# jamie8johnson/cqs

Measured on AMD Instinct MI355X. Metric: queries/sec @k=20 (brute-force cosine scan + top-k, 768-d fp32), higher is better.
Workload: dtype f32; 1 GPU; BASELINE configs[1]: 1000000 x 768 fp32 unit vectors, 1 query per step, brute-force cosine top-20; mode=single, rows_per_gpu=1000000, total_rows=1000000, dim=768, k=20, parallelism=single GPU, ranks_seen=1

## Files before the change

cqs_amd/csrc/scan_bf16.hip:

```cpp
#include "scan_bf16.h"
#include "scan_i8.h"
#include "f32_score.h"
#include "launch_util.h"
#include "rank_sort.h"
#include "scan_gemv_device.h"
#include "select_device.h"
#include "shadow_build_device.h"
#include "tail_plan.h"
#include "tail_prefix.h"

namespace cqs {

static_assert(kShadowKMax == kMaxK, "shadow k' policy and the select agree on max k");

__device__ __forceinline__ float key_score(uint64_t key) {
    const uint32_t ok = (uint32_t)(key >> 32);
    return __uint_as_float((ok & 0x80000000u) ? (ok ^ 0x80000000u) : ~ok);
}

__global__ __launch_bounds__(256) void shadow_build_kernel(const float* __restrict__ rows, uint16_t* __restrict__ shadow,
                                                           uint64_t row0, uint64_t n_rows, uint32_t dim, double gamma,
                                                           unsigned long long* __restrict__ stats) {
    const int lane = threadIdx.x & 63;
    const uint64_t waves = (uint64_t)gridDim.x * (blockDim.x >> 6);
    for (uint64_t r = (uint64_t)blockIdx.x * (blockDim.x >> 6) + (threadIdx.x >> 6); r < n_rows; r += waves) {
        shadow_build_row(rows + (row0 + r) * dim, shadow + (row0 + r) * dim, dim, gamma, stats, lane);
    }
}

hipError_t launch_shadow_build(const float* rows, uint16_t* shadow, uint64_t row0, uint64_t n_rows, uint32_t dim,
                               double gamma, unsigned long long* stats, hipStream_t st) {
    if (n_rows == 0) return hipSuccess;
    const uint64_t blocks = (n_rows + 3u) / 4u;
    hipLaunchKernelGGL(shadow_build_kernel, dim3((uint32_t)(blocks < 8192u ? blocks : 8192u)), dim3(256), 0, st, rows,
                       shadow, row0, n_rows, dim, gamma, stats);
    return hipGetLastError();
}

__global__ __launch_bounds__(64) void shadow_bound_kernel(const float* __restrict__ q, uint32_t dim, double r_max,
                                                          double norm_max, float* __restrict__ bq) {
    const uint32_t lane = threadIdx.x;
    const float v = wave_shadow_bound(q + (size_t)blockIdx.x * dim, dim, r_max, norm_max, lane);
    if (lane == 0) bq[blockIdx.x] = v;
}

hipError_t launch_shadow_bound(const float* q, uint32_t b, uint32_t dim, double r_max, double norm_max, float* bq,
                               hipStream_t st) {
    if (b == 0) return hipSuccess;
    if (b > kShadowMaxQ) return hipErrorInvalidValue;
    hipLaunchKernelGGL(shadow_bound_kernel, dim3(b), dim3(64), 0, st, q, dim, r_max, norm_max, bq);
    return hipGetLastError();
}

struct Bf16ScanParams {
    const uint16_t* rows;
    uint32_t n, n_pad, dim;
    const float* q;
    float* scores;
    const uint32_t* keep;
    uint32_t mode;
    float thr;
    uint32_t nq;
    uint32_t* work;
    TaskTiers tiers;
    uint32_t n_tasks;
    float* gmax;
    uint64_t* gaux;
    const float* bq;
    uint32_t keep_stride;
    uint8_t slot[kMaxGemvQ];
};

template <int NCH, int BQ, int RI, bool NT, bool FULL, bool PQ>
__global__ __launch_bounds__(256) void scan_bf16_kernel(const Bf16ScanParams p) {
    constexpr int NV = RI * BQ;
    constexpr int LPV = 64 / NV;
    const int lane = threadIdx.x & 63;
    const uint32_t n = p.n, dim = p.dim;

    uint32_t coff[NCH];
    f4 qa[BQ][NCH], qb[BQ][NCH];
#pragma unroll
    for (int c = 0; c < NCH; ++c) {
        const uint32_t idx = (uint32_t)c * 512u + (uint32_t)lane * 8u;
        const bool in = FULL || idx < dim;
        coff[c] = in ? idx : dim - 8u;
#pragma unroll
        for (int b = 0; b < BQ; ++b) {
            const float* qp = p.q + (size_t)((uint32_t)b < p.nq ? b : 0) * dim + coff[c];
            const f4 va = *(const f4*)qp, vb = *(const f4*)(qp + 4);
            qa[b][c] = in ? va : (f4)(0.f);
            qb[b][c] = in ? vb : (f4)(0.f);
        }
    }

    const uint32_t last = n - 1u;
    const uint32_t nwords = (n + 31u) / 32u;
    const uint32_t n_tasks = p.n_tasks;
    const uint32_t wpb = blockDim.x >> 6;
    const uint32_t total_waves = gridDim.x * wpb;
    const uint32_t wave_id = (uint32_t)__builtin_amdgcn_readfirstlane((int)(blockIdx.x * wpb + (threadIdx.x >> 6)));
    const bool use_queue = n_tasks > total_waves;
    const uint32_t zero = opaque_zero();

    const char* const rows_b = (const char*)p.rows;
    const uint32_t row_bytes = dim * 2u;
    auto load_rows = [&](uint32_t base, int j, u4 (&x)[RI][NCH]) {
#pragma unroll
        for (int r = 0; r < RI; ++r) {
            uint32_t row = base + (uint32_t)(RI * j + r);
            row = row > last ? last : row;
            const char* rp = rows_b + (uint64_t)row * row_bytes;
#pragma unroll
            for (int c = 0; c < NCH; ++c) {
                const u4* src = (const u4*)(rp + coff[c] * 2u);
                if (NT) x[r][c] = __builtin_nontemporal_load(src);
                else x[r][c] = *src;
            }
        }
        __builtin_amdgcn_sched_barrier(0);
    };
    auto reduce_rows = [&](int j, u4 (&x)[RI][NCH], float (&sc)[BQ]) {
        f2 acc2[NV];
#pragma unroll
        for (int i = 0; i < NV; ++i) acc2[i] = (f2)(0.f);
#pragma unroll
        for (int r = 0; r < RI; ++r)
#pragma unroll
            for (int c = 0; c < NCH; ++c) {
                const u4 w = x[r][c];
                const f2 x0 = {bf_lo(w.x), bf_hi(w.x)}, x1 = {bf_lo(w.y), bf_hi(w.y)};
                const f2 x2 = {bf_lo(w.z), bf_hi(w.z)}, x3 = {bf_lo(w.w), bf_hi(w.w)};
#pragma unroll
                for (int b = 0; b < BQ; ++b) {
                    f2 a = acc2[b * RI + r];
                    a = __builtin_elementwise_fma(x0, __builtin_shufflevector(qa[b][c], qa[b][c], 0, 1), a);
                    a = __builtin_elementwise_fma(x1, __builtin_shufflevector(qa[b][c], qa[b][c], 2, 3), a);
                    a = __builtin_elementwise_fma(x2, __builtin_shufflevector(qb[b][c], qb[b][c], 0, 1), a);
                    a = __builtin_elementwise_fma(x3, __builtin_shufflevector(qb[b][c], qb[b][c], 2, 3), a);
                    acc2[b * RI + r] = a;
                }
            }
        float acc[NV];
#pragma unroll
        for (int i = 0; i < NV; ++i) acc[i] = acc2[i].x + acc2[i].y;
        treduce<NV>(acc, lane);
#pragma unroll
        for (int b = 0; b < BQ; ++b) {
            const float t = __shfl(acc[0], (b * RI + (lane % RI)) * LPV, 64);
            if (lane / RI == j) sc[b] = t;
        }
    };
    uint64_t qmask[PQ ? BQ : 1];
    auto epilogue = [&](uint32_t cur, uint32_t base, uint32_t trows, uint64_t mask, float (&sc)[BQ]) {
        const uint32_t row = base + (uint32_t)lane;
        const bool live_all = (uint32_t)lane < trows && ((mask >> lane) & 1ull);
#pragma unroll
        for (int b = 0; b < BQ; ++b) {
            const bool live = PQ ? (uint32_t)lane < trows && ((qmask[PQ ? b : 0] >> lane) & 1ull) : live_all;
            float s = sc[b];
            if (!live || !(__builtin_fabsf(s) <= 3.4028234664e38f)) s = -INFINITY;
            else if (p.mode == 1u && (uint32_t)b < p.nq) {
                float t = s + p.bq[b];
                t = t < 0.f ? 0.f : (t > 1.f ? 1.f : t);
                if (!(t >= p.thr)) s = -INFINITY;
            }
            if ((uint32_t)b >= p.nq) continue;
            if ((uint32_t)lane < trows && row < p.n_pad) p.scores[(size_t)b * p.n_pad + row] = s;
            const float gm = wave_max64(s);
            if (lane == 0) p.gmax[(size_t)b * n_tasks + cur] = gm;
            if (p.gaux) {
                const uint32_t arg = (uint32_t)__builtin_ctzll(__ballot(s == gm));
                const float sec = wave_max64(((uint32_t)lane == arg) ? -INFINITY : s);
                if (lane == 0) p.gaux[(size_t)b * n_tasks + cur] = ((uint64_t)arg << 32) | (uint64_t)__float_as_uint(sec);
            }
        }
    };
    auto task_mask = [&](uint32_t base, uint32_t trows) -> uint64_t {
        const uint64_t all = trows == 64u ? ~0ull : ((1ull << trows) - 1ull);
        uint64_t mask = all;
        if (base + trows > n) mask = (base >= n) ? 0ull : (all >> (trows - (n - base)));
        if constexpr (PQ) {
            const uint32_t w = base / 32u;
            uint64_t any = 0ull;
#pragma unroll
            for (int b = 0; b < BQ; ++b) {
                uint64_t m = 0ull;
                if ((uint32_t)b < p.nq) {
                    const kc32* kp = (const kc32*)(p.keep + (size_t)p.slot[b] * p.keep_stride);
                    const uint32_t w0 = (w < nwords) ? kp[w] : 0u;
                    const uint32_t w1 = (w + 1u < nwords) ? kp[w + 1u] : 0u;
                    m = mask & ((((uint64_t)w1 << 32) | (uint64_t)w0) >> (base & 31u));
                }
                const uint32_t mlo = __builtin_amdgcn_readfirstlane((uint32_t)m);
                const uint32_t mhi = __builtin_amdgcn_readfirstlane((uint32_t)(m >> 32));
                qmask[b] = ((uint64_t)mhi << 32) | mlo;
                any |= qmask[b];
            }
            return any;
        }
        if (p.keep) {
            const uint32_t w = base / 32u;
            const uint32_t w0 = (w < nwords) ? p.keep[w] : 0u;
            const uint32_t w1 = (w + 1u < nwords) ? p.keep[w + 1u] : 0u;
            mask &= (((uint64_t)w1 << 32) | (uint64_t)w0) >> (base & 31u);
        }
        const uint32_t mlo = __builtin_amdgcn_readfirstlane((uint32_t)mask);
        const uint32_t mhi = __builtin_amdgcn_readfirstlane((uint32_t)(mask >> 32));
        return ((uint64_t)mhi << 32) | mlo;
    };

    u4 x[RI][NCH];
    uint32_t cur = wave_id;
    while (cur < n_tasks) {
        uint32_t trows;
        const uint32_t base = p.tiers.locate(cur, trows);
        const uint64_t mask = task_mask(base, trows);
        uint32_t ticket = 0;
        if (use_queue && lane == 0) ticket = atomicAdd(p.work + zero, 1u);
        float sc[BQ];
#pragma unroll
        for (int b = 0; b < BQ; ++b) sc[b] = -INFINITY;
        const int nb = (int)(trows / (uint32_t)RI);
        for (int j = 0; j < nb; ++j) {
            const uint32_t m = (uint32_t)(mask >> (RI * j)) & ((1u << RI) - 1u);
            if (m == 0u) continue;
            load_rows(base, j, x);
            reduce_rows(j, x, sc);
        }
        epilogue(cur, base, trows, mask, sc);
        cur = use_queue ? total_waves + (uint32_t)__builtin_amdgcn_readfirstlane(ticket) : n_tasks;
    }
}

#ifndef CQS_BF16_ONE_SHOT
#define CQS_BF16_ONE_SHOT 24u
#endif
#ifndef CQS_BF16_BLOCKS_PER_CU
#define CQS_BF16_BLOCKS_PER_CU 2u
#endif

template <int NCH, int BQ, int RI, bool PQ>
static hipError_t launch_bf16(const ScanArgs& a, const uint16_t* shadow, const float* bq, uint32_t q0, uint32_t nq,
                              uint32_t work_slot, hipStream_t st) {
    Bf16ScanParams p;
    fill_gemv_pass(p, a, q0, nq, PQ);
    p.rows = shadow;
    p.work = a.work + work_slot;
    p.bq = bq + q0;
    const bool one_shot = p.n_tasks <= a.n_cu * 4u * CQS_BF16_ONE_SHOT;
    const uint32_t wpb = 4u;
    const uint32_t blocks = one_shot ? (p.n_tasks + wpb - 1u) / wpb : a.n_cu * CQS_BF16_BLOCKS_PER_CU;
    const dim3 grid(blocks), block(64u * wpb);
    const bool full = (a.dim == (uint32_t)NCH * 512u);
    for_nt_full(a.nontemporal, full, [&](auto nt_c, auto full_c) {
        hipLaunchKernelGGL((scan_bf16_kernel<NCH, BQ, RI, decltype(nt_c)::value, decltype(full_c)::value, PQ>), grid, block, 0, st, p);
    });
    return hipGetLastError();
}

template <int NCH, bool PQ>
static hipError_t launch_bf16_groups(const ScanArgs& a, const uint16_t* shadow, const float* bq, hipStream_t st) {
    uint32_t done = 0, slot = 0;
    while (done < a.b) {
        const uint32_t left = a.b - done;
        hipError_t e;
        uint32_t g;
        if constexpr (NCH <= 2) {
            if (left >= 5) { g = left < 8u ? left : 8u; e = launch_bf16<NCH, 8, 2, PQ>(a, shadow, bq, done, g, slot, st); }
            else if (left >= 4) { g = 4; e = launch_bf16<NCH, 4, 4, PQ>(a, shadow, bq, done, g, slot, st); }
            else if (left >= 2) { g = 2; e = launch_bf16<NCH, 2, 8, PQ>(a, shadow, bq, done, g, slot, st); }
            else { g = 1; e = launch_bf16<NCH, 1, 16, PQ>(a, shadow, bq, done, g, slot, st); }
        } else {
            if (left >= 2) { g = 2; e = launch_bf16<NCH, 2, 4, PQ>(a, shadow, bq, done, g, slot, st); }
            else { g = 1; e = launch_bf16<NCH, 1, 8, PQ>(a, shadow, bq, done, g, slot, st); }
        }
        if (e != hipSuccess) return e;
        done += g;
        slot = (slot + 1u) % kWorkWords;
    }
    return hipSuccess;
}

hipError_t launch_scan_bf16(const ScanArgs& a, const uint16_t* shadow, const float* bq, hipStream_t st) {
    if (a.b == 0 || a.n == 0) return hipSuccess;
    if (a.b > kShadowMaxQ || a.dim % 8u != 0u || a.dim > kShadowMaxDim || a.group_tasks != 1u) return hipErrorInvalidValue;
    if (a.keep_tab && !keep_tab_ok(a)) return hipErrorInvalidValue;
    switch ((a.dim + 511u) / 512u) {
        case 1: return a.keep_tab ? launch_bf16_groups<1, true>(a, shadow, bq, st) : launch_bf16_groups<1, false>(a, shadow, bq, st);
        case 2: return a.keep_tab ? launch_bf16_groups<2, true>(a, shadow, bq, st) : launch_bf16_groups<2, false>(a, shadow, bq, st);
        case 3: return a.keep_tab ? launch_bf16_groups<3, true>(a, shadow, bq, st) : launch_bf16_groups<3, false>(a, shadow, bq, st);
        case 4: return a.keep_tab ? launch_bf16_groups<4, true>(a, shadow, bq, st) : launch_bf16_groups<4, false>(a, shadow, bq, st);
        default: return hipErrorInvalidValue;
    }
}

struct TailParams {
    const float* rows;
    const float* q;
    uint32_t dim, k, kprime, mode, row_base;
    float thr;
    const float* scores;
    const float* gmax;
    const uint64_t* gaux;
    uint32_t n_pad;
    TaskTiers tiers;
    uint32_t group_tasks;
    uint32_t bins;
    uint32_t* work;
    uint64_t* ekeys;
    float* bq;
    uint32_t* tickets;
    uint32_t bound;
    double r_max, norm_max;
    uint64_t* out_keys;
    uint32_t* out_counts;
    uint32_t* cert;
    unsigned long long* counters;
    unsigned long long* counters2;
    uint32_t prefix;
    unsigned long long* prefix_counts;
    unsigned long long* dbg;
    uint32_t first;
};

template <int NCH, bool DBG, bool TIER>
__global__ __launch_bounds__(1024) void rescore_certify_kernel(const TailParams p) {
    __shared__ uint64_t s_keys[kShadowKMax];
    __shared__ uint64_t s_sorted[kShadowKMax];
    __shared__ __attribute__((aligned(16))) uint32_t s_ok[kShadowKMax + 4];
    __shared__ uint32_t s_cnt, s_flag, s_last;
    const uint32_t lane = threadIdx.x & 63u;
    const uint32_t qi = blockIdx.y;
    const uint32_t wib = (uint32_t)__builtin_amdgcn_readfirstlane((int)(threadIdx.x >> 6));
    const uint32_t wave = blockIdx.x * kTailWaves + wib;
    const uint32_t n_waves = gridDim.x * kTailWaves;
    const uint32_t dim = p.dim;
    const float* qp = p.q + (size_t)qi * dim;
    unsigned long long* const dbg = DBG && qi == 0u ? p.dbg : nullptr;
#define CQS_TAIL_STAMP(i, who) do { if (DBG && dbg && (who)) dbg[i] = __builtin_amdgcn_s_memrealtime(); } while (0)
    if (threadIdx.x == 0) s_cnt = 0u;
    if (qi == 0u && blockIdx.x == 0u)
        for (uint32_t i = threadIdx.x; i < kWorkWords; i += 1024u) p.work[i] = 0u;
    const GroupMap map{p.tiers, p.group_tasks};
    const uint32_t n_groups = map.total();
    const uint32_t first = TIER ? p.first : 0u;
    uint32_t lim = TIER ? first : p.kprime;
    uint32_t found, ac, nc;
    uint64_t key_next;
    const uint64_t* akeys;
    auto run_select = [&](unsigned long long* stamps) {
        akeys = select_body(p.scores + (size_t)qi * p.n_pad, p.gmax + (size_t)qi * n_groups,
                            p.gaux ? p.gaux + (size_t)qi * n_groups : nullptr, p.n_pad, map, lim + 1u, p.row_base, p.bins,
                            stamps, found);
        found = (uint32_t)__builtin_amdgcn_readfirstlane((int)found);
        ac = found < lim + 1u ? found : lim + 1u;
        nc = ac < lim ? ac : lim;
        key_next = ac > lim ? akeys[lim] : 0ull;
    };
    run_select(DBG ? dbg : nullptr);

    auto write_out = [&](uint32_t m, bool ok) {
        const uint32_t k = p.k;
        const uint32_t outc = m < k ? m : k;
        for (uint32_t i = threadIdx.x; i < k; i += 1024u) p.out_keys[(size_t)qi * k + i] = (i < outc) ? s_sorted[i] : 0ull;
        if (threadIdx.x == 0) {
            p.out_counts[qi] = outc;
            p.cert[qi] = ok ? 1u : 0u;
            if (p.counters) atomicAdd(&p.counters[ok ? 0 : 1], 1ull);
            if (p.counters2) atomicAdd(&p.counters2[ok ? 0 : 1], 1ull);
        }
    };
    auto full_verdict = [&](uint32_t m, float bq) {
        bool ok = false;
        if (__builtin_fabsf(bq) <= 3.4028234664e38f) {
            if (ac <= p.kprime) ok = true;
            else if (m >= p.k) {
                float t = key_score(key_next) + bq;
                if (p.mode == 1u) t = t < 0.f ? 0.f : (t > 1.f ? 1.f : t);
                ok = t < key_score(s_sorted[p.k - 1u]);
// ... 161 lines not shown
```

cqs_amd/csrc/scan_device.h:

```cpp
#pragma once
#include <hip/hip_runtime.h>
#include <stdint.h>

namespace cqs {

typedef float f4 __attribute__((ext_vector_type(4)));
typedef float f2 __attribute__((ext_vector_type(2)));
typedef unsigned u4 __attribute__((ext_vector_type(4)));
typedef __attribute__((address_space(4))) uint32_t kc32;

__device__ __forceinline__ uint32_t okey(float x) {
    uint32_t b = __float_as_uint(x);
    return b ^ ((b >> 31) ? 0xFFFFFFFFu : 0x80000000u);
}
constexpr uint32_t kInvalidKey = 0x007FFFFFu;

__device__ __forceinline__ uint64_t pack_key(uint32_t ok, uint32_t global_row) {
    return ((uint64_t)ok << 32) | (uint64_t)(0xFFFFFFFFu - global_row);
}

template <int N, int M, int NV>
__device__ __forceinline__ void treduce_level(float (&v)[NV], int lane) {
    if constexpr (N > 1) {
        const bool hi = (lane & M) != 0;
#pragma unroll
        for (int i = 0; i < N / 2; ++i) {
            const float keep = hi ? v[i + N / 2] : v[i];
            const float send = hi ? v[i] : v[i + N / 2];
            v[i] = keep + __shfl_xor(send, M, 64);
        }
        treduce_level<N / 2, M / 2, NV>(v, lane);
    } else if constexpr (M >= 1) {
        v[0] += __shfl_xor(v[0], M, 64);
        treduce_level<1, M / 2, NV>(v, lane);
    }
}
template <int NV>
__device__ __forceinline__ void treduce(float (&v)[NV], int lane) {
    treduce_level<NV, 32, NV>(v, lane);
}

}
```

cqs_amd/csrc/scan_i8.hip:

```cpp
#include "scan_i8.h"
#include "launch_util.h"
#include "scan_gemv_device.h"
#include "shadow_build_device.h"

namespace cqs {

template <int I>
__device__ __forceinline__ float code_f32(uint32_t w) { return (float)(int)(int8_t)(w >> (8 * I)); }

__global__ __launch_bounds__(256) void i8_build_kernel(const float* __restrict__ rows, int8_t* __restrict__ codes,
                                                       float* __restrict__ scales, uint64_t row0, uint64_t n_rows,
                                                       uint32_t dim, double gamma, unsigned long long* __restrict__ stats) {
    const uint32_t lane = threadIdx.x & 63u;
    const uint64_t waves = (uint64_t)gridDim.x * (blockDim.x >> 6);
    for (uint64_t r = (uint64_t)blockIdx.x * (blockDim.x >> 6) + (threadIdx.x >> 6); r < n_rows; r += waves) {
        i8_build_row(rows + (row0 + r) * dim, codes + (row0 + r) * dim, scales + row0 + r, dim, gamma, stats, lane);
    }
}

hipError_t launch_i8_build(const float* rows, int8_t* codes, float* scales, uint64_t row0, uint64_t n_rows, uint32_t dim,
                           double gamma, unsigned long long* stats, hipStream_t st) {
    if (n_rows == 0) return hipSuccess;
    if (!i8_dim_ok(dim)) return hipErrorInvalidValue;
    const uint64_t blocks = (n_rows + 3u) / 4u;
    hipLaunchKernelGGL(i8_build_kernel, dim3((uint32_t)(blocks < 8192u ? blocks : 8192u)), dim3(256), 0, st, rows, codes,
                       scales, row0, n_rows, dim, gamma, stats);
    return hipGetLastError();
}

__global__ __launch_bounds__(64) void i8_bound_kernel(const float* __restrict__ q, uint32_t dim, double r_max,
                                                      double norm_max, float* __restrict__ bq) {
    const uint32_t lane = threadIdx.x;
    const float v = wave_i8_bound(q + (size_t)blockIdx.x * dim, dim, r_max, norm_max, lane);
    if (lane == 0) bq[blockIdx.x] = v;
}

hipError_t launch_i8_bound(const float* q, uint32_t b, uint32_t dim, double r_max, double norm_max, float* bq, hipStream_t st) {
    if (b == 0) return hipSuccess;
    if (b > kShadowMaxQ) return hipErrorInvalidValue;
    hipLaunchKernelGGL(i8_bound_kernel, dim3(b), dim3(64), 0, st, q, dim, r_max, norm_max, bq);
    return hipGetLastError();
}

struct I8ScanParams {
    const int8_t* rows;
    const float* scales;
    uint32_t n, n_pad, dim;
    const float* q;
    float* scores;
    const uint32_t* keep;
    uint32_t mode;
    float thr;
    uint32_t nq;
    TaskTiers tiers;
    uint32_t n_tasks;
    float* gmax;
    uint64_t* gaux;
    const float* bq;
    uint32_t keep_stride;
    uint8_t slot[kMaxGemvQ];
    uint32_t group_tasks;
    uint32_t n_groups;
};

constexpr uint32_t kI8BlockWaves = 4;
static_assert(kI8BlockWaves == kMaxGroupTasks, "a workgroup of the int8 scan is one group of the select's map");

template <int NCH, int BQ, int RI, bool NT, bool FULL, bool PQ>
__global__ __launch_bounds__(256) void scan_i8_kernel(const I8ScanParams p) {
    constexpr int NV = RI * BQ;
    constexpr int LPV = 64 / NV;
    __shared__ float s_gmx[kI8BlockWaves][BQ], s_gsec[kI8BlockWaves][BQ];
    __shared__ uint32_t s_garg[kI8BlockWaves][BQ], s_goff[kI8BlockWaves], s_arrive;
    const int lane = threadIdx.x & 63;
    const uint32_t n = p.n, dim = p.dim;
    const bool grouped = p.group_tasks > 1u;
    if (grouped) {
        if (threadIdx.x == 0) s_arrive = 0u;
        __syncthreads();
    }

    uint32_t coff[NCH];
    f4 qv[BQ][NCH][4];
#pragma unroll
    for (int c = 0; c < NCH; ++c) {
        const uint32_t idx = (uint32_t)c * 1024u + (uint32_t)lane * 16u;
        const bool in = FULL || idx < dim;
        coff[c] = in ? idx : dim - 16u;
#pragma unroll
        for (int b = 0; b < BQ; ++b) {
            const float* qp = p.q + (size_t)((uint32_t)b < p.nq ? b : 0) * dim + coff[c];
#pragma unroll
            for (int w = 0; w < 4; ++w) {
                const f4 t = *(const f4*)(qp + 4 * w);
                qv[b][c][w] = in ? t : (f4)(0.f);
            }
        }
    }

    const uint32_t last = n - 1u;
    const uint32_t nwords = (n + 31u) / 32u;
    const uint32_t n_tasks = p.n_tasks;
    const uint32_t wpb = blockDim.x >> 6;
    const uint32_t wib = (uint32_t)__builtin_amdgcn_readfirstlane((int)(threadIdx.x >> 6));
    const uint32_t cur = (uint32_t)__builtin_amdgcn_readfirstlane((int)(blockIdx.x * wpb + (threadIdx.x >> 6)));
    if (cur >= n_tasks) return;

    const char* const rows_b = (const char*)p.rows;
    auto load_rows = [&](uint32_t base, int j, u4 (&x)[RI][NCH]) {
#pragma unroll
        for (int r = 0; r < RI; ++r) {
            uint32_t row = base + (uint32_t)(RI * j + r);
            row = row > last ? last : row;
            const char* rp = rows_b + (uint64_t)row * dim;
#pragma unroll
            for (int c = 0; c < NCH; ++c) {
                const u4* src = (const u4*)(rp + coff[c]);
                if (NT) x[r][c] = __builtin_nontemporal_load(src);
                else x[r][c] = *src;
            }
        }
        __builtin_amdgcn_sched_barrier(0);
    };
    auto reduce_rows = [&](int j, u4 (&x)[RI][NCH], float (&sc)[BQ]) {
        f2 acc2[NV];
#pragma unroll
        for (int i = 0; i < NV; ++i) acc2[i] = (f2)(0.f);
#pragma unroll
        for (int r = 0; r < RI; ++r)
#pragma unroll
            for (int c = 0; c < NCH; ++c)
#pragma unroll
                for (int w = 0; w < 4; ++w) {
                    const uint32_t u = x[r][c][w];
                    const f2 lo = {code_f32<0>(u), code_f32<1>(u)}, hi = {code_f32<2>(u), code_f32<3>(u)};
#pragma unroll
                    for (int b = 0; b < BQ; ++b) {
                        const f4 qq = qv[b][c][w];
                        f2 a = acc2[b * RI + r];
                        a = __builtin_elementwise_fma(lo, __builtin_shufflevector(qq, qq, 0, 1), a);
                        a = __builtin_elementwise_fma(hi, __builtin_shufflevector(qq, qq, 2, 3), a);
                        acc2[b * RI + r] = a;
                    }
                }
        float acc[NV];
#pragma unroll
        for (int i = 0; i < NV; ++i) acc[i] = acc2[i].x + acc2[i].y;
        treduce<NV>(acc, lane);
#pragma unroll
        for (int b = 0; b < BQ; ++b) {
            const float t = __shfl(acc[0], (b * RI + (lane % RI)) * LPV, 64);
            if (lane / RI == j) sc[b] = t;
        }
    };
    uint64_t qmask[PQ ? BQ : 1];
    auto epilogue = [&](uint32_t cur, uint32_t base, uint32_t trows, uint64_t mask, float scale, float (&sc)[BQ]) {
        const uint32_t row = base + (uint32_t)lane;
        const bool live_all = (uint32_t)lane < trows && ((mask >> lane) & 1ull);
#pragma unroll
        for (int b = 0; b < BQ; ++b) {
            const bool live = PQ ? (uint32_t)lane < trows && ((qmask[PQ ? b : 0] >> lane) & 1ull) : live_all;
            float s = sc[b] * scale;
            if (!live || !(__builtin_fabsf(s) <= 3.4028234664e38f)) s = -INFINITY;
            else if (p.mode == 1u && (uint32_t)b < p.nq) {
                float t = s + p.bq[b];
                t = t < 0.f ? 0.f : (t > 1.f ? 1.f : t);
                if (!(t >= p.thr)) s = -INFINITY;
            }
            if ((uint32_t)b >= p.nq) continue;
            if ((uint32_t)lane < trows && row < p.n_pad) p.scores[(size_t)b * p.n_pad + row] = s;
            const float gm = wave_max64(s);
            if (grouped) {
                uint32_t arg = 0u;
                float sec = -INFINITY;
                if (p.gaux) {
                    arg = (uint32_t)__builtin_ctzll(__ballot(s == gm));
                    sec = wave_max64(((uint32_t)lane == arg) ? -INFINITY : s);
                }
                if (lane == 0) { s_gmx[wib][b] = gm; s_garg[wib][b] = arg; s_gsec[wib][b] = sec; }
                continue;
            }
            if (lane == 0) p.gmax[(size_t)b * n_tasks + cur] = gm;
            if (p.gaux) {
                const uint32_t arg = (uint32_t)__builtin_ctzll(__ballot(s == gm));
                const float sec = wave_max64(((uint32_t)lane == arg) ? -INFINITY : s);
                if (lane == 0) p.gaux[(size_t)b * n_tasks + cur] = ((uint64_t)arg << 32) | (uint64_t)__float_as_uint(sec);
            }
        }
        if (!grouped) return;
        const uint32_t g = blockIdx.x;
        uint32_t gr;
        const uint32_t gbase = p.tiers.locate(g * kI8BlockWaves, gr);
        uint32_t t = 0u;
        if (lane == 0) {
            s_goff[wib] = base - gbase;
            t = __hip_atomic_fetch_add(&s_arrive, 1u, __ATOMIC_ACQ_REL, __HIP_MEMORY_SCOPE_WORKGROUP);
        }
        t = (uint32_t)__builtin_amdgcn_readfirstlane((int)t);
        const uint32_t left = n_tasks - g * kI8BlockWaves;
        const uint32_t expect = left < kI8BlockWaves ? left : kI8BlockWaves;
        if (t + 1u != expect) return;
        __builtin_amdgcn_fence(__ATOMIC_ACQUIRE, "workgroup");
        if ((uint32_t)lane < p.nq) {
            MaxTriple w[kI8BlockWaves];
            uint32_t off[kI8BlockWaves];
#pragma unroll
            for (uint32_t i = 0; i < kI8BlockWaves; ++i) {
                const bool there = i < expect;
                w[i] = MaxTriple{there ? s_gmx[i][lane] : -INFINITY, there ? s_garg[i][lane] : 0u, there ? s_gsec[i][lane] : -INFINITY};
                off[i] = there ? s_goff[i] : 0u;
            }
            const MaxTriple m = combine_triples(w, off, kI8BlockWaves);
            p.gmax[(size_t)lane * p.n_groups + g] = m.max;
            if (p.gaux) p.gaux[(size_t)lane * p.n_groups + g] = ((uint64_t)m.arg << 32) | (uint64_t)__float_as_uint(m.sec);
        }
    };
    auto task_mask = [&](uint32_t base, uint32_t trows) -> uint64_t {
        const uint64_t all = trows == 64u ? ~0ull : ((1ull << trows) - 1ull);
        uint64_t mask = all;
        if (base + trows > n) mask = (base >= n) ? 0ull : (all >> (trows - (n - base)));
        if constexpr (PQ) {
            const uint32_t w = base / 32u;
            uint64_t any = 0ull;
#pragma unroll
            for (int b = 0; b < BQ; ++b) {
                uint64_t m = 0ull;
                if ((uint32_t)b < p.nq) {
                    const kc32* kp = (const kc32*)(p.keep + (size_t)p.slot[b] * p.keep_stride);
                    const uint32_t w0 = (w < nwords) ? kp[w] : 0u;
                    const uint32_t w1 = (w + 1u < nwords) ? kp[w + 1u] : 0u;
                    m = mask & ((((uint64_t)w1 << 32) | (uint64_t)w0) >> (base & 31u));
                }
                const uint32_t mlo = __builtin_amdgcn_readfirstlane((uint32_t)m);
                const uint32_t mhi = __builtin_amdgcn_readfirstlane((uint32_t)(m >> 32));
                qmask[b] = ((uint64_t)mhi << 32) | mlo;
                any |= qmask[b];
            }
            return any;
        }
        if (p.keep) {
            const uint32_t w = base / 32u;
            const uint32_t w0 = (w < nwords) ? p.keep[w] : 0u;
            const uint32_t w1 = (w + 1u < nwords) ? p.keep[w + 1u] : 0u;
            mask &= (((uint64_t)w1 << 32) | (uint64_t)w0) >> (base & 31u);
        }
        const uint32_t mlo = __builtin_amdgcn_readfirstlane((uint32_t)mask);
        const uint32_t mhi = __builtin_amdgcn_readfirstlane((uint32_t)(mask >> 32));
        return ((uint64_t)mhi << 32) | mlo;
    };

    u4 x[RI][NCH];
    uint32_t trows;
    const uint32_t base = p.tiers.locate(cur, trows);
    const uint64_t mask = task_mask(base, trows);
    const uint32_t srow = base + (uint32_t)lane;
    const float scale = p.scales[srow > last ? last : srow];
    float sc[BQ];
#pragma unroll
    for (int b = 0; b < BQ; ++b) sc[b] = -INFINITY;
    const int nb = (int)(trows / (uint32_t)RI);
    for (int j = 0; j < nb; ++j) {
        const uint32_t m = (uint32_t)(mask >> (RI * j)) & ((1u << RI) - 1u);
        if (m == 0u) continue;
        load_rows(base, j, x);
        reduce_rows(j, x, sc);
    }
    epilogue(cur, base, trows, mask, scale, sc);
}

constexpr int kI8RowsPerBatch = 16;

template <int NCH, int BQ, int RI, bool PQ>
static hipError_t launch_i8(const ScanArgs& a, const int8_t* codes, const float* scales, const float* bq, uint32_t q0,
                            uint32_t nq, hipStream_t st) {
    I8ScanParams p;
    fill_gemv_pass(p, a, q0, nq, PQ);
    p.rows = codes; p.scales = scales;
    p.bq = bq + q0;
    p.group_tasks = a.group_tasks;
    p.n_groups = (p.n_tasks + a.group_tasks - 1u) / a.group_tasks;
    if (a.group_tasks != 1u) {
        p.gmax = a.gmax + (size_t)q0 * p.n_groups;
        p.gaux = a.gaux ? a.gaux + (size_t)q0 * p.n_groups : nullptr;
    }
    const uint32_t wpb = kI8BlockWaves;
    const dim3 grid((p.n_tasks + wpb - 1u) / wpb), block(64u * wpb);
    const bool full = (a.dim == (uint32_t)NCH * 1024u);
    for_nt_full(a.nontemporal, full, [&](auto nt_c, auto full_c) {
        hipLaunchKernelGGL((scan_i8_kernel<NCH, BQ, RI, decltype(nt_c)::value, decltype(full_c)::value, PQ>), grid, block, 0, st, p);
    });
    return hipGetLastError();
}

template <int NCH, bool PQ>
static hipError_t launch_i8_groups(const ScanArgs& a, const int8_t* codes, const float* scales, const float* bq, hipStream_t st) {
    uint32_t done = 0;
    while (done < a.b) {
        const uint32_t left = a.b - done;
        hipError_t e;
        uint32_t g;
        if (left >= 3) { g = left < 4u ? left : 4u; e = launch_i8<NCH, 4, 4, PQ>(a, codes, scales, bq, done, g, st); }
        else if (left >= 2) { g = 2; e = launch_i8<NCH, 2, 8, PQ>(a, codes, scales, bq, done, g, st); }
        else { g = 1; e = launch_i8<NCH, 1, kI8RowsPerBatch, PQ>(a, codes, scales, bq, done, g, st); }
        if (e != hipSuccess) return e;
        done += g;
    }
    return hipSuccess;
}

hipError_t launch_scan_i8(const ScanArgs& a, const int8_t* codes, const float* scales, const float* bq, hipStream_t st) {
    if (a.b == 0 || a.n == 0) return hipSuccess;
    if (a.b > kShadowMaxQ || !i8_dim_ok(a.dim) || (a.group_tasks != 1u && a.group_tasks != kI8BlockWaves)) return hipErrorInvalidValue;
    if (a.keep_tab && !keep_tab_ok(a)) return hipErrorInvalidValue;
    switch ((a.dim + 1023u) / 1024u) {
        case 1: return a.keep_tab ? launch_i8_groups<1, true>(a, codes, scales, bq, st) : launch_i8_groups<1, false>(a, codes, scales, bq, st);
        case 2: return a.keep_tab ? launch_i8_groups<2, true>(a, codes, scales, bq, st) : launch_i8_groups<2, false>(a, codes, scales, bq, st);
        default: return hipErrorInvalidValue;
    }
}

}
```

cqs_amd/csrc/scan_kernels.hip:

```cpp
#include "scan_kernels.h"
#include "launch_util.h"
#include "scan_gemv_device.h"
#include "select_device.h"

namespace cqs {


struct ScanParams {
    const float* rows;
    uint32_t n, n_pad, dim;
    const float* q;
    float* scores;
    const uint32_t* keep;
    uint32_t mode;
    float thr;
    uint32_t nq;
    uint32_t* work;
    TaskTiers tiers;
    uint32_t n_tasks;
    float* gmax;
    uint64_t* gaux;
    unsigned long long* dbg;
    const uint32_t* gate;
    uint32_t gate_n;
    uint32_t keep_stride;
    uint8_t slot[kMaxGemvQ];
};

template <int NCH, int BQ, int RI, bool NT, bool FULL, int PIPE, int OCC, bool PQ>
__global__ __launch_bounds__(256, OCC) void scan_gemv_kernel(const ScanParams p) {
    if (p.gate && gate_closed(p.gate, p.gate_n)) return;
    constexpr int NV = RI * BQ;
    constexpr int LPV = 64 / NV;
    const int lane = threadIdx.x & 63;
    const uint32_t n = p.n, dim = p.dim;

    uint32_t coff[NCH];
    f4 qv[BQ][NCH];
#pragma unroll
    for (int c = 0; c < NCH; ++c) {
        const uint32_t idx = (uint32_t)c * 256u + (uint32_t)lane * 4u;
        const bool in = FULL || idx < dim;
        coff[c] = in ? idx : dim - 4u;
#pragma unroll
        for (int b = 0; b < BQ; ++b) {
            const f4 v = *(const f4*)(p.q + (size_t)((uint32_t)b < p.nq ? b : 0) * dim + coff[c]);
            qv[b][c] = in ? v : (f4)(0.f);
        }
    }

    const uint32_t last = n - 1u;
    const uint32_t nwords = (n + 31u) / 32u;
    const uint32_t n_tasks = p.n_tasks;
    const uint32_t wpb = blockDim.x >> 6;
    const uint32_t total_waves = gridDim.x * wpb;
    const uint32_t wave_id = (uint32_t)__builtin_amdgcn_readfirstlane((int)(blockIdx.x * wpb + (threadIdx.x >> 6)));
    const bool use_queue = n_tasks > total_waves;
    const uint32_t zero = opaque_zero();
    if (p.dbg && lane == 0 && wave_id < kDbgWaves) p.dbg[16u + 2u * wave_id] = __builtin_amdgcn_s_memrealtime();

    const char* const rows_b = (const char*)p.rows;
    const uint32_t row_bytes = dim * 4u;
    uint32_t lane_off[NCH];
#pragma unroll
    for (int c = 0; c < NCH; ++c) lane_off[c] = coff[c] * 4u;
    auto load_rows = [&](uint32_t base, int j, f4 (&x)[RI][NCH]) {
#pragma unroll
        for (int r = 0; r < RI; ++r) {
            uint32_t row = base + (uint32_t)(RI * j + r);
            row = row > last ? last : row;
            const char* rp = rows_b + (uint64_t)row * row_bytes;
#pragma unroll
            for (int c = 0; c < NCH; ++c) {
                const f4* src = FULL ? (const f4*)(rp + lane_off[0]) + c * 64 : (const f4*)(rp + lane_off[c]);
                if (NT) x[r][c] = __builtin_nontemporal_load(src);
                else x[r][c] = *src;
            }
        }
        __builtin_amdgcn_sched_barrier(0);
    };
    auto reduce_rows = [&](int j, f4 (&x)[RI][NCH], float (&sc)[BQ]) {
        f2 acc2[NV];
#pragma unroll
        for (int i = 0; i < NV; ++i) acc2[i] = (f2)(0.f);
#pragma unroll
        for (int r = 0; r < RI; ++r)
#pragma unroll
            for (int c = 0; c < NCH; ++c) {
                const f2 xlo = __builtin_shufflevector(x[r][c], x[r][c], 0, 1);
                const f2 xhi = __builtin_shufflevector(x[r][c], x[r][c], 2, 3);
#pragma unroll
                for (int b = 0; b < BQ; ++b) {
                    f2 a = acc2[b * RI + r];
                    a = __builtin_elementwise_fma(xlo, __builtin_shufflevector(qv[b][c], qv[b][c], 0, 1), a);
                    a = __builtin_elementwise_fma(xhi, __builtin_shufflevector(qv[b][c], qv[b][c], 2, 3), a);
                    acc2[b * RI + r] = a;
                }
            }
        float acc[NV];
#pragma unroll
        for (int i = 0; i < NV; ++i) acc[i] = acc2[i].x + acc2[i].y;
        treduce<NV>(acc, lane);
#pragma unroll
        for (int b = 0; b < BQ; ++b) {
            const float t = __shfl(acc[0], (b * RI + (lane % RI)) * LPV, 64);
            if (lane / RI == j) sc[b] = t;
        }
    };

    uint64_t qmask[PQ ? BQ : 1];
    auto epilogue = [&](uint32_t cur, uint32_t base, uint32_t trows, uint64_t mask, float (&sc)[BQ]) {
        const uint32_t row = base + (uint32_t)lane;
        bool live = (uint32_t)lane < trows && ((mask >> lane) & 1ull);
#pragma unroll
        for (int b = 0; b < BQ; ++b) {
            float s = sc[b];
            if constexpr (PQ) live = (uint32_t)lane < trows && ((qmask[b] >> lane) & 1ull);
            if (!live || !(__builtin_fabsf(s) <= 3.4028234664e38f)) s = -INFINITY;
            else if (p.mode == 1u) {
                s = s < 0.f ? 0.f : (s > 1.f ? 1.f : s);
                if (!(s >= p.thr)) s = -INFINITY;
            }
            if ((uint32_t)b >= p.nq) continue;
            if ((uint32_t)lane < trows && row < p.n_pad) p.scores[(size_t)b * p.n_pad + row] = s;
            const float gm = wave_max64(s);
            if (lane == 0) p.gmax[(size_t)b * n_tasks + cur] = gm;
            if (p.gaux) {
                const uint32_t arg = (uint32_t)__builtin_ctzll(__ballot(s == gm));
                const float sec = wave_max64(((uint32_t)lane == arg) ? -INFINITY : s);
                if (lane == 0) p.gaux[(size_t)b * n_tasks + cur] = ((uint64_t)arg << 32) | (uint64_t)__float_as_uint(sec);
            }
        }
    };
    auto claimed = [&](uint32_t ticket) -> uint32_t {
        return use_queue ? total_waves + (uint32_t)__builtin_amdgcn_readfirstlane(ticket) : n_tasks;
    };

    auto task_mask = [&](uint32_t base, uint32_t trows) -> uint64_t {
        const uint64_t all = trows == 64u ? ~0ull : ((1ull << trows) - 1ull);
        uint64_t mask = all;
        if (base + trows > n) mask = (base >= n) ? 0ull : (all >> (trows - (n - base)));
        if constexpr (PQ) {
            const uint32_t w = base / 32u;
            uint64_t any = 0ull;
#pragma unroll
            for (int b = 0; b < BQ; ++b) {
                uint64_t m = 0ull;
                if ((uint32_t)b < p.nq) {
                    const kc32* kp = (const kc32*)(p.keep + (size_t)p.slot[b] * p.keep_stride);
                    const uint32_t w0 = (w < nwords) ? kp[w] : 0u;
                    const uint32_t w1 = (w + 1u < nwords) ? kp[w + 1u] : 0u;
                    m = mask & ((((uint64_t)w1 << 32) | (uint64_t)w0) >> (base & 31u));
                }
                const uint32_t mlo = __builtin_amdgcn_readfirstlane((uint32_t)m);
                const uint32_t mhi = __builtin_amdgcn_readfirstlane((uint32_t)(m >> 32));
                qmask[b] = ((uint64_t)mhi << 32) | mlo;
                any |= qmask[b];
            }
            return any;
        }
        if (p.keep) {
            const uint32_t w = base / 32u;
            const uint32_t w0 = (w < nwords) ? p.keep[w] : 0u;
            const uint32_t w1 = (w + 1u < nwords) ? p.keep[w + 1u] : 0u;
            mask &= (((uint64_t)w1 << 32) | (uint64_t)w0) >> (base & 31u);
        }
        const uint32_t mlo = __builtin_amdgcn_readfirstlane((uint32_t)mask);
        const uint32_t mhi = __builtin_amdgcn_readfirstlane((uint32_t)(mask >> 32));
        return ((uint64_t)mhi << 32) | mlo;
    };
    f4 xa[RI][NCH], xb[RI][NCH];
    auto sparse_task = [&](uint32_t t, uint32_t base, uint32_t trows, uint64_t mask) {
        float sc[BQ];
#pragma unroll
        for (int b = 0; b < BQ; ++b) sc[b] = -INFINITY;
        const int nb = (int)(trows / (uint32_t)RI);
        for (int j = 0; j < nb; ++j) {
            const uint32_t m = (uint32_t)(mask >> (RI * j)) & ((1u << RI) - 1u);
            if (m == 0u) continue;
            load_rows(base, j, xb);
            reduce_rows(j, xb, sc);
        }
        epilogue(t, base, trows, mask, sc);
    };

    uint32_t cur = wave_id;
    while (cur < n_tasks) {
        uint32_t trows;
        const uint32_t base = p.tiers.locate(cur, trows);
        const uint64_t mask = task_mask(base, trows);
        const uint64_t all = trows == 64u ? ~0ull : ((1ull << trows) - 1ull);
        uint32_t ticket = 0;
        if (PIPE == 1 && mask == all) {
            float sc[BQ];
#pragma unroll
            for (int b = 0; b < BQ; ++b) sc[b] = -INFINITY;
            const int steps = (int)(trows / (2u * (uint32_t)RI));
            load_rows(base, 0, xa);
            for (int s = 0; s < steps; ++s) {
                load_rows(base, 2 * s + 1, xb);
                if (s == 0 && use_queue && lane == 0) ticket = atomicAdd(p.work + zero, 1u);
                reduce_rows(2 * s, xa, sc);
                if (s + 1 < steps) load_rows(base, 2 * s + 2, xa);
                reduce_rows(2 * s + 1, xb, sc);
            }
            epilogue(cur, base, trows, mask, sc);
        } else {
            if (use_queue && lane == 0) ticket = atomicAdd(p.work + zero, 1u);
            sparse_task(cur, base, trows, mask);
        }
        cur = claimed(ticket);
    }
    if (p.dbg && lane == 0 && wave_id < kDbgWaves) p.dbg[17u + 2u * wave_id] = __builtin_amdgcn_s_memrealtime();
}

__global__ __launch_bounds__(1024) void select_finish_kernel(const float* __restrict__ scores,
                                                             const float* __restrict__ gmax,
                                                             const uint64_t* __restrict__ gaux, uint32_t n_pad,
                                                             const TaskTiers tiers, uint32_t slot_log2, uint32_t k,
                                                             uint32_t row_base, uint32_t linear,
                                                             uint64_t* __restrict__ out_keys,
                                                             uint32_t* __restrict__ out_counts,
                                                             uint32_t* __restrict__ work,
                                                             unsigned long long* __restrict__ dbg,
                                                             const uint32_t* __restrict__ gate, uint32_t gate_n) {
    if (gate && gate_closed(gate, gate_n)) return;
    const uint32_t qi = blockIdx.x;
    const uint32_t n_tasks = tiers.total();
    uint32_t count;
    const uint64_t* sorted = select_body(scores + (size_t)qi * n_pad, gmax + (size_t)qi * n_tasks,
                                         gaux ? gaux + (size_t)qi * n_tasks : nullptr, n_pad, GroupMap{tiers, 1u}, k, row_base, linear, dbg,
                                         count);
    const uint32_t outc = count < k ? count : k;
    for (uint32_t i = threadIdx.x; i < k; i += 1024u) out_keys[(size_t)qi * k + i] = (i < outc) ? sorted[i] : 0ull;
    if (threadIdx.x == 0) out_counts[qi] = outc;
    if (qi == 0) for (uint32_t i = threadIdx.x; i < kWorkWords; i += 1024u) work[i] = 0u;
    if (dbg && threadIdx.x == 0 && blockIdx.x == 0) dbg[6] = __builtin_amdgcn_s_memrealtime();
}

bool scan_dim_supported(uint32_t dim) { return dim >= 4 && dim % 4 == 0 && dim <= 4096; }

#ifndef CQS_SCAN_PIPE
#define CQS_SCAN_PIPE 1
#endif
#ifndef CQS_SCAN_RI1
#define CQS_SCAN_RI1 8
#endif
#ifndef CQS_SCAN_CAP_OCCUPANCY
#define CQS_SCAN_CAP_OCCUPANCY 1
#endif
#ifndef CQS_SCAN_ONE_SHOT
#define CQS_SCAN_ONE_SHOT 24u
#endif
#ifndef CQS_SCAN_BLOCK_WAVES
#define CQS_SCAN_BLOCK_WAVES 2u
// ... 147 lines not shown
```

cqs_amd/csrc/wave_ops.h:

```cpp
#pragma once
#if defined(__HIPCC__)
#include <hip/hip_runtime.h>
namespace cqs {
typedef unsigned lane_u2 __attribute__((ext_vector_type(2)));
__device__ __forceinline__ lane_u2 swap16_self(unsigned x) { return __builtin_amdgcn_permlane16_swap(x, x, false, false); }
__device__ __forceinline__ lane_u2 swap32_self(unsigned x) { return __builtin_amdgcn_permlane32_swap(x, x, false, false); }

template <int CTRL>
__device__ __forceinline__ float wave_dpp(float v) {
    return __builtin_bit_cast(float, __builtin_amdgcn_update_dpp(0, __builtin_bit_cast(int, v), CTRL, 0xF, 0xF, false));
}

__device__ __forceinline__ float xor16_max(float v) {
    const lane_u2 a = swap16_self(__float_as_uint(v));
    return fmaxf(__uint_as_float(a[0]), __uint_as_float(a[1]));
}
__device__ __forceinline__ float xor32_max(float v) {
    const lane_u2 a = swap32_self(__float_as_uint(v));
    return fmaxf(__uint_as_float(a[0]), __uint_as_float(a[1]));
}
__device__ __forceinline__ float xor16_sum(float v) {
    const lane_u2 a = swap16_self(__float_as_uint(v));
    return __uint_as_float(a[0]) + __uint_as_float(a[1]);
}
__device__ __forceinline__ float xor32_sum(float v) {
    const lane_u2 a = swap32_self(__float_as_uint(v));
    return __uint_as_float(a[0]) + __uint_as_float(a[1]);
}
__device__ __forceinline__ float xor32_value(float v, int lane) {
    const lane_u2 a = swap32_self(__float_as_uint(v));
    return __uint_as_float(lane < 32 ? a[1] : a[0]);
}

__device__ __forceinline__ float wave_max16(float m) {
    m = fmaxf(m, wave_dpp<0xB1>(m));
    m = fmaxf(m, wave_dpp<0x4E>(m));
    m = fmaxf(m, wave_dpp<0x141>(m));
    m = fmaxf(m, wave_dpp<0x140>(m));
    return m;
}
__device__ __forceinline__ float half_wave_max(float m) { return xor16_max(wave_max16(m)); }
__device__ __forceinline__ float wave_max64(float m) { return xor32_max(xor16_max(wave_max16(m))); }

__device__ __forceinline__ float wave_sum16(float v) {
    v += wave_dpp<0xB1>(v);
    v += wave_dpp<0x4E>(v);
    v += wave_dpp<0x141>(v);
    v += wave_dpp<0x140>(v);
    return v;
}
__device__ __forceinline__ float half_wave_sum32(float v) { return xor16_sum(wave_sum16(v)); }
__device__ __forceinline__ float row_sum_of_halves(float v) { return xor32_sum(half_wave_sum32(v)); }
__device__ __forceinline__ float wave_sum64_readlane(float v) {
    const int b = __builtin_bit_cast(int, wave_sum16(v));
    return __builtin_bit_cast(float, __builtin_amdgcn_readlane(b, 0)) + __builtin_bit_cast(float, __builtin_amdgcn_readlane(b, 16)) +
           __builtin_bit_cast(float, __builtin_amdgcn_readlane(b, 32)) + __builtin_bit_cast(float, __builtin_amdgcn_readlane(b, 48));
}
__device__ __forceinline__ float wave_sum64_shfl(float v) {
#pragma unroll
    for (int off = 32; off >= 1; off >>= 1) v += __shfl_xor(v, off, 64);
    return v;
}
__device__ __forceinline__ double wave_sum64_shfl(double v) {
#pragma unroll
    for (int off = 32; off >= 1; off >>= 1) v += __shfl_xor(v, off, 64);
    return v;
}
}
#endif
```

Before: 6892 queries/s.

## Use scalar row bases, DPP/permlane reductions, and unclamped full-block loads in scans

Row addresses in the bf16 and int8 scan loaders are made wave-uniform through readfirstlane so they can sit in scalar registers with per-lane vector offsets, and row clamping is skipped unless the block crosses the end. The butterfly tree reduction swaps __shfl_xor (LDS bpermute) for permlane32/16 swaps and DPP row operations that fold two values per step. The int8 kernel also gets a fixed waves-per-EU occupancy hint. These target address arithmetic and cross-lane traffic in the inner GEMV loop, at the cost of more intricate DPP mask logic that has to be correct for every NV.

```diff
diff --git a/cqs_amd/csrc/scan_bf16.hip b/cqs_amd/csrc/scan_bf16.hip
--- a/cqs_amd/csrc/scan_bf16.hip
+++ b/cqs_amd/csrc/scan_bf16.hip
@@ -105,15 +105,23 @@
 
     const char* const rows_b = (const char*)p.rows;
     const uint32_t row_bytes = dim * 2u;
-    auto load_rows = [&](uint32_t base, int j, u4 (&x)[RI][NCH]) {
+    auto load_rows = [&](uint32_t base, int j, u4 (&x)[RI][NCH], auto clamp_c) {
+        uint32_t off[NCH];
+#pragma unroll
+        for (int c = 0; c < NCH; ++c) off[c] = lane_offset(coff[c] * 2u);
+        const uint32_t row0 = base + (uint32_t)(RI * j);
+        const char* const bp = rows_b + (uint64_t)row0 * row_bytes;
 #pragma unroll
         for (int r = 0; r < RI; ++r) {
-            uint32_t row = base + (uint32_t)(RI * j + r);
-            row = row > last ? last : row;
-            const char* rp = rows_b + (uint64_t)row * row_bytes;
+            const char* up = bp + (uint32_t)r * row_bytes;
+            if constexpr (decltype(clamp_c)::value) {
+                const uint32_t row = row0 + (uint32_t)r;
+                up = rows_b + (uint64_t)(row > last ? last : row) * row_bytes;
+            }
+            const gchar* rp = scalar_global(up);
 #pragma unroll
             for (int c = 0; c < NCH; ++c) {
-                const u4* src = (const u4*)(rp + coff[c] * 2u);
+                const gu4* src = (const gu4*)(rp + off[c]);
                 if (NT) x[r][c] = __builtin_nontemporal_load(src);
                 else x[r][c] = *src;
             }
@@ -144,7 +152,7 @@
         float acc[NV];
 #pragma unroll
         for (int i = 0; i < NV; ++i) acc[i] = acc2[i].x + acc2[i].y;
-        treduce<NV>(acc, lane);
+        treduce<NV>(acc);
 #pragma unroll
         for (int b = 0; b < BQ; ++b) {
             const float t = __shfl(acc[0], (b * RI + (lane % RI)) * LPV, 64);
@@ -225,7 +233,8 @@
         for (int j = 0; j < nb; ++j) {
             const uint32_t m = (uint32_t)(mask >> (RI * j)) & ((1u << RI) - 1u);
             if (m == 0u) continue;
-            load_rows(base, j, x);
+            if (base + (uint32_t)(RI * (j + 1)) > n) load_rows(base, j, x, std::true_type{});
+            else load_rows(base, j, x, std::false_type{});
             reduce_rows(j, x, sc);
         }
         epilogue(cur, base, trows, mask, sc);
diff --git a/cqs_amd/csrc/scan_device.h b/cqs_amd/csrc/scan_device.h
--- a/cqs_amd/csrc/scan_device.h
+++ b/cqs_amd/csrc/scan_device.h
@@ -1,6 +1,7 @@
 #pragma once
 #include <hip/hip_runtime.h>
 #include <stdint.h>
+#include "wave_ops.h"
 
 namespace cqs {
 
@@ -8,6 +9,20 @@
 typedef float f2 __attribute__((ext_vector_type(2)));
 typedef unsigned u4 __attribute__((ext_vector_type(4)));
 typedef __attribute__((address_space(4))) uint32_t kc32;
+
+typedef __attribute__((address_space(1))) char gchar;
+typedef __attribute__((address_space(1))) u4 gu4;
+__device__ __forceinline__ const gchar* scalar_global(const void* p) {
+    const uint64_t x = (uint64_t)p;
+    const uint32_t lo = (uint32_t)__builtin_amdgcn_readfirstlane((int)(uint32_t)x);
+    const uint32_t hi = (uint32_t)__builtin_amdgcn_readfirstlane((int)(uint32_t)(x >> 32));
+    return (const gchar*)(((uint64_t)hi << 32) | lo);
+}
+
+__device__ __forceinline__ uint32_t lane_offset(uint32_t off) {
+    asm volatile("" : "+v"(off));
+    return off;
+}
 
 __device__ __forceinline__ uint32_t okey(float x) {
     uint32_t b = __float_as_uint(x);
@@ -20,24 +35,30 @@
 }
 
 template <int N, int M, int NV>
-__device__ __forceinline__ void treduce_level(float (&v)[NV], int lane) {
+__device__ __forceinline__ void treduce_level(float (&v)[NV]) {
     if constexpr (N > 1) {
-        const bool hi = (lane & M) != 0;
+        static_assert(M >= 4, "a fold below distance 4 has no bank mask: at most 16 values per wave");
 #pragma unroll
         for (int i = 0; i < N / 2; ++i) {
-            const float keep = hi ? v[i + N / 2] : v[i];
-            const float send = hi ? v[i] : v[i + N / 2];
-            v[i] = keep + __shfl_xor(send, M, 64);
+            if constexpr (M == 32) v[i] = fold32_sum(v[i], v[i + N / 2]);
+            else if constexpr (M == 16) v[i] = fold16_sum(v[i], v[i + N / 2]);
+            else if constexpr (M == 8) v[i] = fold8_sum(v[i], v[i + N / 2]);
+            else v[i] = fold4_sum(v[i], v[i + N / 2]);
         }
-        treduce_level<N / 2, M / 2, NV>(v, lane);
+        treduce_level<N / 2, M / 2, NV>(v);
     } else if constexpr (M >= 1) {
-        v[0] += __shfl_xor(v[0], M, 64);
-        treduce_level<1, M / 2, NV>(v, lane);
+        if constexpr (M == 32) v[0] = xor32_sum(v[0]);
+        else if constexpr (M == 16) v[0] = xor16_sum(v[0]);
+        else if constexpr (M == 8) v[0] = xor8_sum(v[0]);
+        else if constexpr (M == 4) v[0] = fold4_sum(v[0], v[0]);
+        else if constexpr (M == 2) v[0] = xor2_sum(v[0]);
+        else v[0] = xor1_sum(v[0]);
+        treduce_level<1, M / 2, NV>(v);
     }
 }
 template <int NV>
-__device__ __forceinline__ void treduce(float (&v)[NV], int lane) {
-    treduce_level<NV, 32, NV>(v, lane);
+__device__ __forceinline__ void treduce(float (&v)[NV]) {
+    treduce_level<NV, 32, NV>(v);
 }
 
 }
diff --git a/cqs_amd/csrc/scan_i8.hip b/cqs_amd/csrc/scan_i8.hip
--- a/cqs_amd/csrc/scan_i8.hip
+++ b/cqs_amd/csrc/scan_i8.hip
@@ -67,7 +67,7 @@
 static_assert(kI8BlockWaves == kMaxGroupTasks, "a workgroup of the int8 scan is one group of the select's map");
 
 template <int NCH, int BQ, int RI, bool NT, bool FULL, bool PQ>
-__global__ __launch_bounds__(256) void scan_i8_kernel(const I8ScanParams p) {
+__global__ __launch_bounds__(256) __attribute__((amdgpu_waves_per_eu(4, 4))) void scan_i8_kernel(const I8ScanParams p) {
     constexpr int NV = RI * BQ;
     constexpr int LPV = 64 / NV;
     __shared__ float s_gmx[kI8BlockWaves][BQ], s_gsec[kI8BlockWaves][BQ];
@@ -107,15 +107,23 @@
     if (cur >= n_tasks) return;
 
     const char* const rows_b = (const char*)p.rows;
-    auto load_rows = [&](uint32_t base, int j, u4 (&x)[RI][NCH]) {
+    auto load_rows = [&](uint32_t base, int j, u4 (&x)[RI][NCH], auto clamp_c) {
+        uint32_t off[NCH];
+#pragma unroll
+        for (int c = 0; c < NCH; ++c) off[c] = lane_offset(coff[c]);
+        const uint32_t row0 = base + (uint32_t)(RI * j);
+        const char* const bp = rows_b + (uint64_t)row0 * dim;
 #pragma unroll
         for (int r = 0; r < RI; ++r) {
-            uint32_t row = base + (uint32_t)(RI * j + r);
-            row = row > last ? last : row;
-            const char* rp = rows_b + (uint64_t)row * dim;
+            const char* up = bp + (uint32_t)r * dim;
+            if constexpr (decltype(clamp_c)::value) {
+                const uint32_t row = row0 + (uint32_t)r;
+                up = rows_b + (uint64_t)(row > last ? last : row) * dim;
+            }
+            const gchar* rp = scalar_global(up);
 #pragma unroll
             for (int c = 0; c < NCH; ++c) {
-                const u4* src = (const u4*)(rp + coff[c]);
+                const gu4* src = (const gu4*)(rp + off[c]);
                 if (NT) x[r][c] = __builtin_nontemporal_load(src);
                 else x[r][c] = *src;
             }
@@ -146,7 +154,7 @@
         float acc[NV];
 #pragma unroll
         for (int i = 0; i < NV; ++i) acc[i] = acc2[i].x + acc2[i].y;
-        treduce<NV>(acc, lane);
+        treduce<NV>(acc);
 #pragma unroll
         for (int b = 0; b < BQ; ++b) {
             const float t = __shfl(acc[0], (b * RI + (lane % RI)) * LPV, 64);
@@ -262,7 +270,8 @@
     for (int j = 0; j < nb; ++j) {
         const uint32_t m = (uint32_t)(mask >> (RI * j)) & ((1u << RI) - 1u);
         if (m == 0u) continue;
-        load_rows(base, j, x);
+        if (base + (uint32_t)(RI * (j + 1)) > n) load_rows(base, j, x, std::true_type{});
+        else load_rows(base, j, x, std::false_type{});
         reduce_rows(j, x, sc);
     }
     epilogue(cur, base, trows, mask, scale, sc);
diff --git a/cqs_amd/csrc/scan_kernels.hip b/cqs_amd/csrc/scan_kernels.hip
--- a/cqs_amd/csrc/scan_kernels.hip
+++ b/cqs_amd/csrc/scan_kernels.hip
@@ -100,7 +100,7 @@
         float acc[NV];
 #pragma unroll
         for (int i = 0; i < NV; ++i) acc[i] = acc2[i].x + acc2[i].y;
-        treduce<NV>(acc, lane);
+        treduce<NV>(acc);
 #pragma unroll
         for (int b = 0; b < BQ; ++b) {
             const float t = __shfl(acc[0], (b * RI + (lane % RI)) * LPV, 64);
diff --git a/cqs_amd/csrc/wave_ops.h b/cqs_amd/csrc/wave_ops.h
--- a/cqs_amd/csrc/wave_ops.h
+++ b/cqs_amd/csrc/wave_ops.h
@@ -31,6 +31,25 @@
     const lane_u2 a = swap32_self(__float_as_uint(v));
     return __uint_as_float(lane < 32 ? a[1] : a[0]);
 }
+
+__device__ __forceinline__ float fold32_sum(float a, float b) {
+    const lane_u2 r = __builtin_amdgcn_permlane32_swap(__float_as_uint(a), __float_as_uint(b), false, false);
+    return __uint_as_float(r[0]) + __uint_as_float(r[1]);
+}
+__device__ __forceinline__ float fold16_sum(float a, float b) {
+    const lane_u2 r = __builtin_amdgcn_permlane16_swap(__float_as_uint(a), __float_as_uint(b), false, false);
+    return __uint_as_float(r[0]) + __uint_as_float(r[1]);
+}
+template <int ROR_LO, int ROR_HI, int BANKS_HI>
+__device__ __forceinline__ float fold_row_sum(float a, float b) {
+    const float lo = a + wave_dpp<0x120 + ROR_LO>(a), hi = b + wave_dpp<0x120 + ROR_HI>(b);
+    return __builtin_bit_cast(float, __builtin_amdgcn_update_dpp(__builtin_bit_cast(int, lo), __builtin_bit_cast(int, hi), 0xE4, 0xF, BANKS_HI, false));
+}
+__device__ __forceinline__ float fold8_sum(float a, float b) { return fold_row_sum<8, 8, 0xC>(a, b); }
+__device__ __forceinline__ float fold4_sum(float a, float b) { return fold_row_sum<12, 4, 0xA>(a, b); }
+__device__ __forceinline__ float xor8_sum(float v) { return v + wave_dpp<0x128>(v); }
+__device__ __forceinline__ float xor2_sum(float v) { return v + wave_dpp<0x4E>(v); }
+__device__ __forceinline__ float xor1_sum(float v) { return v + wave_dpp<0xB1>(v); }
 
 __device__ __forceinline__ float wave_max16(float m) {
     m = fmaxf(m, wave_dpp<0xB1>(m));
```

Result: no change. 6940 queries/s, median of 3 (+0.7%).
